# seagochen/unet-segment-pytorch

Hardware: AMD Instinct MI355X
Metric: 512x512 CT slices/sec fwd+bwd, AttentionUNet bs=4/GPU, 1/2/4/8 MI355X (higher is better)
Workload: dtype bf16; 1 GPU; attention_unet 1x512x512 train step (fwd+DiceBCE+bwd+clip+AdamW); model=attention_unet, global_batch=4, per_gpu_batch=4, grad_accum=1, parallelism=single

## Files before the change

### unet-segment-pytorch_amd/csrc/misc.hip

```cpp
#include "halo_items.h"

namespace unet {

__device__ __forceinline__ void up_range(float scale, int i, int in_size, int up, int& lo, int& hi) {
  if (scale > 0.f) {
    lo = (int)floorf((float)(i - 1) / scale) - 1;
    hi = (int)ceilf((float)(i + 1) / scale) + 1;
    lo = lo < 0 ? 0 : lo;
    hi = hi > up - 1 ? up - 1 : hi;
  } else {
    lo = 0;
    hi = up - 1;
  }
}
__device__ __forceinline__ float up_weight(float scale, int u, int in_size, int i) {
  int i0, i1;
  float l;
  lin_idx(scale, u, in_size, i0, i1, l);
  return (i0 == i ? 1.f - l : 0.f) + (i1 == i ? l : 0.f);
}

__global__ void upsample_bwd4_kernel(long long N, int C, int Hs, int Ws, int up_h, int up_w, int pt, int pl, int Hp,
                                     int Wp, float sh, float sw, const float* dup, float* dx, int accum) {
  const int C4 = C / 4;
// ... 93 lines not shown
                                                                int ntj, int ntc) {
  __shared__ float4 t[UPB_VMAX][UPB_CT];
  __shared__ int tab_i0[UPB_VMAX], tab_i1[UPB_VMAX];
  __shared__ float tab_l[UPB_VMAX];
  const int tid = threadIdx.x;
  const unsigned lb = xcd_block(blockIdx.x, gridDim.x);
  const int ct = (int)(lb % (unsigned)ntc);
  unsigned r = lb / (unsigned)ntc;
  const int jt = (int)(r % (unsigned)ntj);
  r /= (unsigned)ntj;
  const int i = (int)(r % (unsigned)Hs);
  const int n = (int)(r / (unsigned)Hs);
  const int C4 = C >> 2, c4 = ct * UPB_CT + (tid & (UPB_CT - 1));
  const int j0 = jt * UPB_J;
  const int ulo = max(0, (int)ceilf((float)(i - 1) / sh) - 1), uhi = min(up_h - 1, (int)floorf((float)(i + 1) / sh) + 1);
  float wy[8];
#pragma unroll
  for (int k = 0; k < 8; ++k) {
    const int u = ulo + k, yy = u + pt;
    wy[k] = (u <= uhi && yy >= 0 && yy < Hp) ? up_weight(sh, u, Hs, i) : 0.f;
  }
  const int jlast = min(Ws - 1, j0 + UPB_J - 1);
  const int vlo = max(0, (int)ceilf((float)(j0 - 1) / sw) - 1), vhi = min(up_w - 1, (int)floorf((float)(jlast + 1) / sw) + 1);
  const int nv = vhi - vlo + 1;
  if (tid < nv) {
    const int v = vlo + tid, xx = v + pl;
    int a0, a1;
    float l;
    lin_idx(sw, v, Ws, a0, a1, l);
    const bool ok = xx >= 0 && xx < Wp;
    tab_i0[tid] = ok ? a0 : -1;
    tab_i1[tid] = ok ? a1 : -1;
    tab_l[tid] = l;
  }
  const bool cok = c4 < C4;
  const size_t rowpix = (size_t)Wp * C4;
  const float4* base = reinterpret_cast<const float4*>(dup) + ((size_t)n * Hp + (ulo + pt)) * rowpix + c4;
  for (int it = tid >> 4; it < nv; it += 256 / UPB_CT) {
    const int xx = vlo + it + pl;
    float4 a = make_float4(0.f, 0.f, 0.f, 0.f);
    if (cok && xx >= 0 && xx < Wp) {
      const float4* p = base + (size_t)xx * C4;
      float4 g[8];
#pragma unroll
      for (int k = 0; k < 8; ++k) g[k] = wy[k] != 0.f ? p[(size_t)k * rowpix] : make_float4(0.f, 0.f, 0.f, 0.f);
#pragma unroll
      for (int k = 0; k < 8; ++k) {
        a.x = __builtin_fmaf(wy[k], g[k].x, a.x); a.y = __builtin_fmaf(wy[k], g[k].y, a.y);
        a.z = __builtin_fmaf(wy[k], g[k].z, a.z); a.w = __builtin_fmaf(wy[k], g[k].w, a.w);
      }
    }
    t[it][tid & (UPB_CT - 1)] = a;
  }
  __syncthreads();
  const int j = j0 + (tid >> 4);
  if (j > jlast || !cok) return;
  const int vjlo = max(vlo, (int)ceilf((float)(j - 1) / sw) - 1), vjhi = min(vhi, (int)floorf((float)(j + 1) / sw) + 1);
  float4 a = make_float4(0.f, 0.f, 0.f, 0.f);
  for (int v = vjlo; v <= vjhi; ++v) {
    const int q = v - vlo;
    const float l = tab_l[q];
    const float w = (tab_i0[q] == j ? 1.f - l : 0.f) + (tab_i1[q] == j ? l : 0.f);
    const float4 g = t[q][tid & (UPB_CT - 1)];
    a.x = __builtin_fmaf(w, g.x, a.x); a.y = __builtin_fmaf(w, g.y, a.y);
    a.z = __builtin_fmaf(w, g.z, a.z); a.w = __builtin_fmaf(w, g.w, a.w);
  }
  float4* o = reinterpret_cast<float4*>(dx) + (((size_t)n * Hs + i) * Ws + j) * C4 + c4;
  if (accum) {
    const float4 b = *o;
    a.x += b.x; a.y += b.y; a.z += b.z; a.w += b.w;
  }
  *o = a;
}

constexpr unsigned UPB_OOB = 0x40000000u;
typedef __amdgpu_buffer_rsrc_t upb_rsrc_t;
__device__ __forceinline__ upb_rsrc_t upb_rsrc(const void* p, unsigned bytes) {
  return __builtin_amdgcn_make_buffer_rsrc(const_cast<void*>(p), (short)0, (int)bytes, 0x00020000);
}
__device__ __forceinline__ uint4 upb_ld(upb_rsrc_t r, unsigned voff, unsigned soff) {
  return __builtin_bit_cast(uint4, __builtin_amdgcn_raw_buffer_load_b128(r, (int)voff, (int)soff, 0));
}

template <typename T, int NCH, int WA>
__global__ __launch_bounds__(256, 4) void upsample_bwd_pw_kernel(int N, int C, int Hs, int Ws, int up_h, int up_w, int pt,
                                                              int pl, int Hp, int Wp, float sh, float sw,
                                                              const float* __restrict__ dup,
                                                              const uint4* __restrict__ dgw,
                                                              const uint4* __restrict__ wt, float* dx, int accum,
                                                              int ntj, int ntc) {
  typedef typename Mma<T>::frag F;
  __shared__ float4 t[UPB_VMAX][UPB_CT + 1];
  __shared__ int tab_i0[UPB_VMAX], tab_i1[UPB_VMAX];
  __shared__ float tab_l[UPB_VMAX];
  const int tid = threadIdx.x, lane = tid & 63, wave = tid >> 6, i16 = lane & 15, g = lane >> 4;
  const unsigned lb = xcd_block(blockIdx.x, gridDim.x);
  const int ct = (int)(lb % (unsigned)ntc);
  unsigned r = lb / (unsigned)ntc;
  const int jt = (int)(r % (unsigned)ntj);
  r /= (unsigned)ntj;
  const int i = (int)(r % (unsigned)Hs);
  const int n = (int)(r / (unsigned)Hs);
  const int C4 = C >> 2;
  const int j0 = jt * UPB_J;
  const int ulo = max(0, (int)ceilf((float)(i - 1) / sh) - 1), uhi = min(up_h - 1, (int)floorf((float)(i + 1) / sh) + 1);
  float wy[8];
#pragma unroll
  for (int k = 0; k < 8; ++k) {
    const int u = ulo + k, yy = u + pt;
    wy[k] = (u <= uhi && yy >= 0 && yy < Hp) ? up_weight(sh, u, Hs, i) : 0.f;
  }
  const int jlast = min(Ws - 1, j0 + UPB_J - 1);
  const int vlo = max(0, (int)ceilf((float)(j0 - 1) / sw) - 1), vhi = min(up_w - 1, (int)floorf((float)(jlast + 1) / sw) + 1);
  const int nv = vhi - vlo + 1;
  if (tid < nv) {
    const int v = vlo + tid, xx = v + pl;
    int a0, a1;
    float l;
    lin_idx(sw, v, Ws, a0, a1, l);
    const bool ok = xx >= 0 && xx < Wp;
    tab_i0[tid] = ok ? a0 : -1;
    tab_i1[tid] = ok ? a1 : -1;
    tab_l[tid] = l;
  }
  const int wa = wave % (4 / WA), wg = wave / (4 / WA);
  F wq[WA][NCH];
#pragma unroll
  for (int aa = 0; aa < WA; ++aa)
#pragma unroll
    for (int c = 0; c < NCH; ++c)
      wq[aa][c] = __builtin_bit_cast(F, wt[((size_t)(ct * 4 + wa * WA + aa) * NCH + c) * 64 + lane]);
  const int cl = 4 * wa * WA + g;
  const size_t img = (size_t)Hp * Wp;
  const upb_rsrc_t dr = upb_rsrc(dup + (size_t)n * img * C, (unsigned)(img * C * 4));
  const upb_rsrc_t xr = upb_rsrc(dgw + (size_t)n * img * (4 * NCH), (unsigned)(img * (64 * NCH)));
  int nlive = 0, pos[8];
#pragma unroll
  for (int k = 0; k < 8; ++k) pos[k] = wy[k] != 0.f ? nlive++ : -1;
  float wl[8];
  unsigned rowd[8], rowx[8];
#pragma unroll
  for (int j = 0; j < 8; ++j) {
    wl[j] = 0.f;
    unsigned row = 0u;
#pragma unroll
    for (int k = 0; k < 8; ++k)
      if (pos[k] == j) { wl[j] = wy[k]; row = (unsigned)(ulo + k + pt) * (unsigned)Wp; }
    rowd[j] = row * (unsigned)C * 4u;
    rowx[j] = row * (unsigned)(64 * NCH);
  }
  const float4 z4 = make_float4(0.f, 0.f, 0.f, 0.f);
  for (int it = 16 * wg + i16; it - i16 < nv; it += 16 * WA) {
    const int xx = vlo + it + pl;
    const bool ok = it < nv && xx >= 0 && xx < Wp;
    const unsigned dvo = ok ? (unsigned)xx * (unsigned)C * 4u + (unsigned)(ct * UPB_CT + cl) * 16u : UPB_OOB;
    const unsigned xvo = ok ? (unsigned)xx * (unsigned)(64 * NCH) + (unsigned)g * 16u : UPB_OOB;
    float4 a[WA];
#pragma unroll
    for (int aa = 0; aa < WA; ++aa) a[aa] = z4;
#pragma unroll
    for (int k0 = 0; k0 < 8; k0 += 4) {
      if (k0 && nlive <= 4) break;
      float4 dv[WA][4];
      f32x4 acc[WA][4];
      unsigned dvk[4], xvk[4];
#pragma unroll
      for (int k = 0; k < 4; ++k) {
        const bool live = k0 + k < nlive;
        dvk[k] = live ? dvo : UPB_OOB;
        xvk[k] = live ? xvo : UPB_OOB;
#pragma unroll
        for (int aa = 0; aa < WA; ++aa) {
          dv[aa][k] = __builtin_bit_cast(float4, upb_ld(dr, dvk[k], rowd[k0 + k] + (unsigned)aa * 64u));
          acc[aa][k] = f32x4{0.f, 0.f, 0.f, 0.f};
        }
      }
#pragma unroll
      for (int c = 0; c < NCH; ++c) {
        uint4 q[4];
#pragma unroll
        for (int k = 0; k < 4; ++k) q[k] = upb_ld(xr, xvk[k], rowx[k0 + k] + (unsigned)c * 64u);
#pragma unroll
        for (int aa = 0; aa < WA; ++aa)
#pragma unroll
          for (int k = 0; k < 4; ++k)
            acc[aa][k] = Mma<T>::mma(wq[aa][c], __builtin_bit_cast(F, q[k]), acc[aa][k]);
      }
#pragma unroll
      for (int aa = 0; aa < WA; ++aa)
#pragma unroll
        for (int k = 0; k < 4; ++k) {
          float4 v = make_float4(acc[aa][k][0], acc[aa][k][1], acc[aa][k][2], acc[aa][k][3]);
          v.x += dv[aa][k].x; v.y += dv[aa][k].y; v.z += dv[aa][k].z; v.w += dv[aa][k].w;
          const float w = wl[k0 + k];
          a[aa].x = __builtin_fmaf(w, v.x, a[aa].x); a[aa].y = __builtin_fmaf(w, v.y, a[aa].y);
          a[aa].z = __builtin_fmaf(w, v.z, a[aa].z); a[aa].w = __builtin_fmaf(w, v.w, a[aa].w);
        }
    }
    if (it < nv) {
#pragma unroll
      for (int aa = 0; aa < WA; ++aa) t[it][cl + 4 * aa] = a[aa];
    }
  }
  __syncthreads();
  const int j = j0 + (tid >> 4);
  if (j > jlast) return;
  const int c4 = ct * UPB_CT + (tid & (UPB_CT - 1));
  const int vjlo = max(vlo, (int)ceilf((float)(j - 1) / sw) - 1), vjhi = min(vhi, (int)floorf((float)(j + 1) / sw) + 1);
  float4 a = z4;
  for (int v = vjlo; v <= vjhi; ++v) {
    const int q = v - vlo;
    const float l = tab_l[q];
    const float w = (tab_i0[q] == j ? 1.f - l : 0.f) + (tab_i1[q] == j ? l : 0.f);
    const float4 gq = t[q][tid & (UPB_CT - 1)];
    a.x = __builtin_fmaf(w, gq.x, a.x); a.y = __builtin_fmaf(w, gq.y, a.y);
    a.z = __builtin_fmaf(w, gq.z, a.z); a.w = __builtin_fmaf(w, gq.w, a.w);
  }
  float4* o = reinterpret_cast<float4*>(dx) + (((size_t)n * Hs + i) * Ws + j) * C4 + c4;
  if (accum) {
    const float4 b = *o;
    a.x += b.x; a.y += b.y; a.z += b.z; a.w += b.w;
  }
  *o = a;
}

template <typename T>
static void launch_upb_pw(int nch, unsigned nblk, hipStream_t st, int N, int C, int Hs, int Ws, int up_h, int up_w,
                          int pt, int pl, int Hp, int Wp, float sh, float sw, const float* d_up, const void* dgw,
                          const void* wt, float* dx, int accum, int ntj, int ntc) {
  const uint4* x = (const uint4*)dgw;
  const uint4* w = (const uint4*)wt;
  const char* e = getenv("UNET_GUP_WA");
  const int wa = e ? atoi(e) : 2;
#define UPB_PW_LAUNCH_WA(NCH, WA)                                                                                      \
  hipLaunchKernelGGL((upsample_bwd_pw_kernel<T, NCH, WA>), dim3(nblk), dim3(256), 0, st, N, C, Hs, Ws, up_h, up_w, pt, \
                     pl, Hp, Wp, sh, sw, d_up, x, w, dx, accum, ntj, ntc)
#define UPB_PW_LAUNCH(NCH)                   \
  do {                                       \
    if (wa == 2) UPB_PW_LAUNCH_WA(NCH, 2);   \
    else UPB_PW_LAUNCH_WA(NCH, 1);           \
  } while (0)
  if (nch == 1) UPB_PW_LAUNCH(1);
  else if (nch == 2) UPB_PW_LAUNCH(2);
  else if (nch == 4) UPB_PW_LAUNCH_WA(4, 1);
  else UPB_PW_LAUNCH_WA(8, 1);
#undef UPB_PW_LAUNCH
#undef UPB_PW_LAUNCH_WA
}

__global__ void upsample_bwd_kernel(long long N, int C, int Hs, int Ws, int up_h, int up_w, int pt, int pl, int Hp,
                                    int Wp, float sh, float sw, const float* dup, float* dx, int accum) {
  const long long total = N * Hs * (long long)Ws * C;
  for (long long e = blockIdx.x * (long long)blockDim.x + threadIdx.x; e < total; e += (long long)gridDim.x * blockDim.x) {
    const int c = e % C;
    long long t = e / C;
    const int j = t % Ws;
    t /= Ws;
    const int i = t % Hs;
    const long long n = t / Hs;
    int ulo, uhi, vlo, vhi;
    up_range(sh, i, Hs, up_h, ulo, uhi);
    up_range(sw, j, Ws, up_w, vlo, vhi);
    float acc = 0.f;
    for (int u = ulo; u <= uhi; ++u) {
      const float wy = up_weight(sh, u, Hs, i);
      if (wy == 0.f) continue;
      const int yy = u + pt;
      if (yy < 0 || yy >= Hp) continue;
      float racc = 0.f;
      for (int v = vlo; v <= vhi; ++v) {
        const float wx = up_weight(sw, v, Ws, j);
        if (wx == 0.f) continue;
        const int xx = v + pl;
        if (xx < 0 || xx >= Wp) continue;
        racc += wx * dup[((n * Hp + yy) * (long long)Wp + xx) * C + c];
      }
      acc += wy * racc;
    }
    dx[e] = accum ? dx[e] + acc : acc;
  }
}

__global__ void resize_nchw_kernel(long long NC, int Hi, int Wi, int Ho, int Wo, float sh, float sw, const float* x,
                                   float* y) {
  const long long total = NC * Ho * (long long)Wo;
  for (long long e = blockIdx.x * (long long)blockDim.x + threadIdx.x; e < total; e += (long long)gridDim.x * blockDim.x) {
    const int v = e % Wo;
    long long t = e / Wo;
    const int u = t % Ho;
    const long long nc = t / Ho;
    int y0, y1, x0, x1;
    float ly, lx;
    lin_idx(sh, u, Hi, y0, y1, ly);
    lin_idx(sw, v, Wi, x0, x1, lx);
    const float* p = x + nc * Hi * (long long)Wi;
    const float a = p[y0 * Wi + x0], b = p[y0 * Wi + x1], c = p[y1 * Wi + x0], d = p[y1 * Wi + x1];
    y[e] = (1.f - ly) * ((1.f - lx) * a + lx * b) + ly * ((1.f - lx) * c + lx * d);
  }
}

__global__ void resize_nchw_bwd_kernel(long long NC, int Hi, int Wi, int Ho, int Wo, float sh, float sw, const float* dy,
                                       float* dx, int accum) {
  const long long total = NC * Hi * (long long)Wi;
  for (long long e = blockIdx.x * (long long)blockDim.x + threadIdx.x; e < total; e += (long long)gridDim.x * blockDim.x) {
    const int j = e % Wi;
    long long t = e / Wi;
    const int i = t % Hi;
    const long long nc = t / Hi;
    int ulo, uhi, vlo, vhi;
    up_range(sh, i, Hi, Ho, ulo, uhi);
    up_range(sw, j, Wi, Wo, vlo, vhi);
    const float* p = dy + nc * Ho * (long long)Wo;
    float acc = 0.f;
    for (int u = ulo; u <= uhi; ++u) {
      const float wy = up_weight(sh, u, Hi, i);
      if (wy == 0.f) continue;
      float racc = 0.f;
      for (int v = vlo; v <= vhi; ++v) {
        const float wx = up_weight(sw, v, Wi, j);
        if (wx != 0.f) racc += wx * p[u * (long long)Wo + v];
      }
      acc += wy * racc;
    }
    dx[e] = accum ? dx[e] + acc : acc;
  }
}

constexpr int OC_MAXK = 8;

template <typename T>
// ... 649 lines not shown
  const I stride = (I)gridDim.x * blockDim.x;
  I e = (I)blockIdx.x * blockDim.x + threadIdx.x;
  const int cv = (int)(e & (CV - 1));
  float sc[VEC], sf[VEC];
#pragma unroll
  for (int j = 0; j < VEC; ++j) { sc[j] = s.scale[cv * VEC + j]; sf[j] = s.shift[cv * VEC + j]; }
  const float lo = s.relu ? 0.f : -INFINITY;
  for (; e < total; e += stride) {
    const I px = e >> cvs;
    const I t = px / (I)W;
    const int x = (int)(px - t * (I)W);
    const I t2 = t / (I)H;
    const int y = (int)(t - t2 * (I)H);
    const long long n = (long long)t2;
    float best[VEC];
    int arg[VEC];
#pragma unroll
    for (int q = 0; q < 4; ++q) {
      float v[VEC];
      load_vec<T>((const T*)s.data + (((n * s.H + 2 * y + (q >> 1)) * (long long)s.W + 2 * x + (q & 1)) * C + cv * VEC), v);
#pragma unroll
      for (int j = 0; j < VEC; ++j) {
        const float r = __builtin_fmaf(v[j], sc[j], sf[j]);
        const float a = r != r ? r : fmaxf(r, lo);
        if (q == 0 || a > best[j] || a != a) { best[j] = a; arg[j] = q; }
      }
    }
    store_vec<T>(out + (size_t)px * C + cv * VEC, best);
    unsigned lo4 = 0, hi4 = 0;
#pragma unroll
    for (int j = 0; j < 4; ++j) lo4 |= (unsigned)arg[j] << (8 * j);
    if constexpr (VEC == 8) {
#pragma unroll
      for (int j = 0; j < 4; ++j) hi4 |= (unsigned)arg[4 + j] << (8 * j);
      *reinterpret_cast<uint2*>(code + (size_t)px * C + cv * VEC) = make_uint2(lo4, hi4);
    } else {
      *reinterpret_cast<unsigned*>(code + (size_t)px * C + cv * VEC) = lo4;
    }
  }
}

}

using namespace unet;

extern "C" {

int unet_upsample_bwd(long long N, int C, int Hs, int Ws, int up_h, int up_w, int pad_t, int pad_l, int Hp, int Wp,
                      float sh, float sw, const float* d_up, float* dx, int accum, void* stream) {
  const long long total = N * Hs * (long long)Ws * C;
  auto span = [](float sc, int up) { return sc > 0.f ? (int)floorf(2.f / sc) + 3 : up + 8; };
  if (C % 4 == 0 && span(sh, up_h) <= 8 && span(sw, up_w) <= 8) {
    const int vspan = (int)floorf((float)(UPB_J + 1) / sw) + 4;
    const char* e = getenv("UNET_UPB_TILE");
    const long long ntj = cdiv(Ws, UPB_J), ntc = cdiv(C / 4, UPB_CT), nblk = N * Hs * ntj * ntc;
    if (!(e && atoi(e) == 0) && vspan <= UPB_VMAX && nblk < (1LL << 31)) {
      hipLaunchKernelGGL(upsample_bwd_tile_kernel, dim3((unsigned)nblk), dim3(256), 0, (hipStream_t)stream, (int)N, C, Hs,
                         Ws, up_h, up_w, pad_t, pad_l, Hp, Wp, sh, sw, d_up, dx, accum, (int)ntj, (int)ntc);
      return check_launch("upsample_bwd");
    }
    if (total / 4 < (1LL << 31))
      hipLaunchKernelGGL(upsample_bwd4w_kernel<unsigned>, dim3(grid_for(total / 4, block_cap("UNET_UPB_BLOCKS", 8192))), dim3(256), 0, (hipStream_t)stream,
                         N, C, Hs, Ws, up_h, up_w, pad_t, pad_l, Hp, Wp, sh, sw, d_up, dx, accum);
    else
      hipLaunchKernelGGL(upsample_bwd4w_kernel<unsigned long long>, dim3(grid_for(total / 4, block_cap("UNET_UPB_BLOCKS", 8192))), dim3(256), 0,
                         (hipStream_t)stream, N, C, Hs, Ws, up_h, up_w, pad_t, pad_l, Hp, Wp, sh, sw, d_up, dx, accum);
    return check_launch("upsample_bwd");
  }
  if (C % 4 == 0) {
    hipLaunchKernelGGL(upsample_bwd4_kernel, dim3(grid_for(total / 4, block_cap("UNET_UPB_BLOCKS", 8192))), dim3(256), 0, (hipStream_t)stream, N, C, Hs,
                       Ws, up_h, up_w, pad_t, pad_l, Hp, Wp, sh, sw, d_up, dx, accum);
    return check_launch("upsample_bwd");
  }
  hipLaunchKernelGGL(upsample_bwd_kernel, dim3(grid_for(total)), dim3(256), 0, (hipStream_t)stream, N, C, Hs, Ws,
                     up_h, up_w, pad_t, pad_l, Hp, Wp, sh, sw, d_up, dx, accum);
  return check_launch("upsample_bwd");
}

int unet_upsample_bwd_pw_ok(int dtype, long long N, int C, int Hs, int Ws, int up_h, int up_w, int pad_t, int pad_l,
                            int Hp, int Wp, float sh, float sw, int Ci) {
  if (dtype != UNET_BF16 && dtype != UNET_F16) return 0;
  if (N < 1 || C < 64 || C % 64 || (Ci != 32 && Ci != 64 && Ci != 128 && Ci != 256)) return 0;
  if (Hs < 1 || Ws < 1 || up_h < 1 || up_w < 1 || Hp < 1 || Wp < 1) return 0;
  auto span = [](float sc, int up) { return sc > 0.f ? (int)floorf(2.f / sc) + 3 : up + 8; };
  if (span(sh, up_h) > 8 || span(sw, up_w) > 8) return 0;
  const int vspan = (int)floorf((float)(UPB_J + 1) / sw) + 4;
  const char* e = getenv("UNET_UPB_TILE");
  const long long nblk = N * Hs * (long long)cdiv(Ws, UPB_J) * (C / 64);
  if ((e && atoi(e) == 0) || vspan > UPB_VMAX || nblk >= (1LL << 31) || N * Hs >= (1LL << 31)) return 0;
  const double img = (double)Hp * Wp;
  return img * C * 4 < (double)UPB_OOB && img * Ci * 2 < (double)UPB_OOB;
}

int unet_upsample_bwd_pw(int dtype, long long N, int C, int Hs, int Ws, int up_h, int up_w, int pad_t, int pad_l,
                         int Hp, int Wp, float sh, float sw, const float* d_up, const void* dgw, int Ci,
                         const void* wt_packed, float* dx, int accum, void* stream) {
  if (!unet_upsample_bwd_pw_ok(dtype, N, C, Hs, Ws, up_h, up_w, pad_t, pad_l, Hp, Wp, sh, sw, Ci)) {
    set_error("unet_upsample_bwd_pw: geometry not served (unet_upsample_bwd_pw_ok)");
    return -1;
  }
  const int ntj = cdiv(Ws, UPB_J), ntc = C / 64;
  const unsigned nblk = (unsigned)(N * Hs * ntj * ntc);
  if (dtype == UNET_F16)
    launch_upb_pw<f16>(Ci / 32, nblk, (hipStream_t)stream, (int)N, C, Hs, Ws, up_h, up_w, pad_t, pad_l, Hp, Wp, sh, sw,
                       d_up, dgw, wt_packed, dx, accum, ntj, ntc);
  else
    launch_upb_pw<bf16>(Ci / 32, nblk, (hipStream_t)stream, (int)N, C, Hs, Ws, up_h, up_w, pad_t, pad_l, Hp, Wp, sh, sw,
                        d_up, dgw, wt_packed, dx, accum, ntj, ntc);
  return check_launch("upsample_bwd_pw");
}

int unet_resize_nchw(long long NC, int Hi, int Wi, int Ho, int Wo, float sh, float sw, const float* x, float* y,
                     void* stream) {
  hipLaunchKernelGGL(resize_nchw_kernel, dim3(grid_for(NC * Ho * (long long)Wo)), dim3(256), 0, (hipStream_t)stream,
                     NC, Hi, Wi, Ho, Wo, sh, sw, x, y);
  return check_launch("resize_nchw");
}

int unet_resize_nchw_bwd(long long NC, int Hi, int Wi, int Ho, int Wo, float sh, float sw, const float* dy, float* dx,
                         int accum, void* stream) {
  hipLaunchKernelGGL(resize_nchw_bwd_kernel, dim3(grid_for(NC * Hi * (long long)Wi)), dim3(256), 0,
                     (hipStream_t)stream, NC, Hi, Wi, Ho, Wo, sh, sw, dy, dx, accum);
  return check_launch("resize_nchw_bwd");
}

int unet_outconv_rows(long long P) { return oc_rows(P); }

int unet_outconv_fwd(int dtype, long long N, int H, int W, int C, int K, const void* y, const float* scale,
                     const float* shift, int relu, const float* w, const float* b, float* logits, void* stream) {
  if (K > OC_MAXK || K < 1) { set_error("unet_outconv_fwd: n_classes > 8 unsupported"); return UNET_ERR_UNSUPPORTED; }
  const long long P = N * H * (long long)W;
  const int G = (C % 8 == 0 && C / 8 <= 64 && ((C / 8) & (C / 8 - 1)) == 0) ? C / 8 : 0;
  if (G && K == 2) {
    long long blocks = (P * G + 255) / 256;
    if (blocks > 4096) blocks = 4096;
    if (dtype == UNET_F16)
      hipLaunchKernelGGL((outconv_fwd_vec_kernel<f16, 2>), dim3((int)blocks), dim3(256), 0, (hipStream_t)stream, P,
                         H * W, C, G, (const f16*)y, scale, shift, relu, w, b, logits);
    else if (dtype == UNET_BF16)
      hipLaunchKernelGGL((outconv_fwd_vec_kernel<bf16, 2>), dim3((int)blocks), dim3(256), 0, (hipStream_t)stream, P,
                         H * W, C, G, (const bf16*)y, scale, shift, relu, w, b, logits);
    else
      hipLaunchKernelGGL((outconv_fwd_vec_kernel<float, 2>), dim3((int)blocks), dim3(256), 0, (hipStream_t)stream, P,
                         H * W, C, G, (const float*)y, scale, shift, relu, w, b, logits);
    return check_launch("outconv_fwd");
  }
  const size_t shm = (size_t)(K * C + 2 * C) * sizeof(float);
  if (dtype == UNET_F16)
    hipLaunchKernelGGL(outconv_fwd_kernel<f16>, dim3(grid_for(P)), dim3(256), shm, (hipStream_t)stream, P, H * W, C, K,
                       (const f16*)y, scale, shift, relu, w, b, logits);
  else if (dtype == UNET_BF16)
    hipLaunchKernelGGL(outconv_fwd_kernel<bf16>, dim3(grid_for(P)), dim3(256), shm, (hipStream_t)stream, P, H * W, C, K,
                       (const bf16*)y, scale, shift, relu, w, b, logits);
  else
    hipLaunchKernelGGL(outconv_fwd_kernel<float>, dim3(grid_for(P)), dim3(256), shm, (hipStream_t)stream, P, H * W, C,
                       K, (const float*)y, scale, shift, relu, w, b, logits);
  return check_launch("outconv_fwd");
}

int unet_outconv_bwd(int dtype, long long N, int H, int W, int C, int K, const void* y, const float* scale,
                     const float* shift, int relu, const float* w, const float* dl, float* da, int accum, float* partial,
                     void* stream) {
  if (K > OC_MAXK || K < 1 || C < K) { set_error("unet_outconv_bwd: need 1 <= n_classes <= min(8, C)"); return UNET_ERR_UNSUPPORTED; }
  const long long P = N * H * (long long)W;
  const int cl = chan_lanes_m(C), rows = oc_rows(P);
  const int G = (C % 8 == 0 && C / 8 <= 256 && ((C / 8) & (C / 8 - 1)) == 0) ? C / 8 : 0;
  if (dtype != UNET_F32 && G && K == 2) {
    if (dtype == UNET_F16)
      hipLaunchKernelGGL((outconv_bwd_vec_kernel<f16, 2>), dim3(rows), dim3(256), 0, (hipStream_t)stream, P, H * W, C, G,
                         (const f16*)y, scale, shift, relu, w, dl, da, accum, partial);
    else
      hipLaunchKernelGGL((outconv_bwd_vec_kernel<bf16, 2>), dim3(rows), dim3(256), 0, (hipStream_t)stream, P, H * W, C, G,
                         (const bf16*)y, scale, shift, relu, w, dl, da, accum, partial);
    return check_launch("outconv_bwd");
  }
  dim3 grid(cdiv(C, cl), rows);
  if (dtype == UNET_F16)
    hipLaunchKernelGGL(outconv_bwd_kernel<f16>, grid, dim3(256), 0, (hipStream_t)stream, P, H * W, C, cl, K,
                       (const f16*)y, scale, shift, relu, w, dl, da, accum, partial, rows);
  else if (dtype == UNET_BF16)
    hipLaunchKernelGGL(outconv_bwd_kernel<bf16>, grid, dim3(256), 0, (hipStream_t)stream, P, H * W, C, cl, K,
                       (const bf16*)y, scale, shift, relu, w, dl, da, accum, partial, rows);
  else
    hipLaunchKernelGGL(outconv_bwd_kernel<float>, grid, dim3(256), 0, (hipStream_t)stream, P, H * W, C, cl, K,
                       (const float*)y, scale, shift, relu, w, dl, da, accum, partial, rows);
  return check_launch("outconv_bwd");
}

int unet_outconv_bwd_bn(int dtype, long long N, int H, int W, int C, int K, const void* y, const float* scale,
                        const float* shift, int relu, const float* w, const float* dl, const float* mean,
                        const float* invstd, float* partial, float* bn_partial, void* stream) {
// ... 218 lines not shown
```

### unet-segment-pytorch_amd/unet/_hip/stages.py

```python

from __future__ import annotations

import os
from typing import Dict, List, Optional

import torch

from . import lib as L
from .runtime import (Act, Precision, conv_kernel_name, f32, pack_many, pack_weight, probe, stream, up_scale, vp,
                      wgrad_kernel_name)


def _conv_desc(prec: Precision, N: int, H: int, W: int, cin: int, cout: int, k: int, srcs: List[L.Src],
               weight: torch.Tensor) -> L.ConvDesc:
    d = L.ConvDesc()
    d.dtype = prec.code
    d.N, d.H, d.W, d.Cin, d.Cout, d.ksize = N, H, W, cin, cout, k
    d.nsrc = len(srcs)
    for i, s in enumerate(srcs):
        d.src[i] = s
    d.weight = weight.data_ptr()
    return d


# ... 311 lines not shown
        wg = self.cg.pre_wp if self.cg.pre_wp is not None else pack_weight(self.cg.conv.weight, prec, False)
        wx = self.cx.pre_wp if self.cx.pre_wp is not None else pack_weight(self.cx.conv.weight, prec, False)
        self.cg.pre_wp = self.cx.pre_wp = None
        gab, xab = f32(2, ci, device=dev), f32(2, ci, device=dev)
        for bn, ab in ((self.cg.bn, gab), (self.cx.bn, xab)):
            L.call("unet_bn_eval_affine", ci, vp(bn.weight), vp(bn.bias), vp(bn.running_mean), vp(bn.running_var),
                   float(bn.eps), vp(ab[0]), vp(ab[1]), None, None, stream())
        self.wpsi = self.psi_conv.weight.detach().reshape(-1).float().contiguous()
        self.p = f32(x.N, x.H, x.W, device=dev)
        L.call("unet_gate_psi_eval", prec.code, x.pixels, g_up_t.shape[-1], x.C, ci, vp(g_up_t), vp(x.data),
               vp(x.ab[0]), vp(x.ab[1]), int(x.relu), vp(wg), vp(wx), vp(gab), vp(xab), vp(self.wpsi),
               vp(self.p), stream())
        bn = self.psi_bn
        self.psi_ab = f32(2, 1, device=dev)
        L.call("unet_bn_eval_affine", 1, vp(bn.weight), vp(bn.bias), vp(bn.running_mean), vp(bn.running_var),
               float(bn.eps), vp(self.psi_ab[0]), vp(self.psi_ab[1]), None, None, stream())

    def gated_src(self) -> L.Src:
        return self.x.src_gated(self.p, self.psi_ab)

    def backward(self, prec, d_xs: torch.Tensor, grads: Grads, d_gup: Optional[torch.Tensor], d_gup_accum: int,
                 defer_g: bool = False):
        x = self.x
        dev = x.data.device
        P, Cx, Ci = x.pixels, x.C, self.ci
        fuse = self._wx_gated_ok(prec, x)
        dx, dx_acc = (None, 0) if fuse else x.grad_target()
        dq = f32(P, device=dev)
        rows1 = L.load().unet_gate_psi_rows(P)
        part1 = f32(2, rows1, device=dev)
        L.call("unet_gate_bwd1", prec.code, P, Cx, vp(d_xs), vp(x.data), vp(x.ab[0]), vp(x.ab[1]), int(x.relu), vp(self.p),
               vp(self.psi_ab), vp(self.psi_mean), vp(self.psi_invstd), vp(dx), dx_acc, vp(dq), vp(part1), stream())
        dgp, dbp, pcoef = f32(1, device=dev), f32(1, device=dev), f32(3, device=dev)
        L.call("unet_bn_bwd_finalize", vp(part1[0]), vp(part1[1]), rows1, 1, P if self.psi_batch else 0,
               vp(self.psi_bn.weight),
               vp(self.psi_mean), vp(self.psi_invstd), vp(dgp), vp(dbp), 0, vp(pcoef), stream())
        grads.put(self.psi_bn.weight, dgp)
        grads.put(self.psi_bn.bias, dbp)
        rows2 = L.load().unet_gate_bwd2_rows(P, Ci)
        part2 = f32(4, rows2, Ci, device=dev)
        L.call("unet_gate_bwd2", prec.code, P, Ci, vp(self.gw.data), vp(self.xw.data), vp(self.gw.ab),
               vp(self.xw.ab), vp(self.gw.mean), vp(self.gw.invstd), vp(self.xw.mean), vp(self.xw.invstd),
               vp(self.wpsi), vp(dq), vp(self.p), vp(pcoef), vp(part2), stream())
        dgg, dbg, gcoef = f32(Ci, device=dev), f32(Ci, device=dev), f32(3, Ci, device=dev)
        dgx, dbx, xcoef = f32(Ci, device=dev), f32(Ci, device=dev), f32(3, Ci, device=dev)
        dwpsi = f32(Ci, device=dev)
        jobs = [_bwd_fin_job(part2[0], part2[1], rows2, Ci, P if self.gw.batch_stats else 0, self.cg.bn.weight,
                             self.gw.mean, self.gw.invstd, dgg, dbg, gcoef),
                _bwd_fin_job(part2[0], part2[2], rows2, Ci, P if self.xw.batch_stats else 0, self.cx.bn.weight,
                             self.xw.mean, self.xw.invstd, dgx, dbx, xcoef),
                _bwd_fin_job(part2[3], None, rows2, Ci, 0, None, None, None, None, dwpsi, None)]
        L.call("unet_bn_bwd_finalize_multi", len(jobs), (L.BnBwdFinJob * len(jobs))(*jobs), stream())
        grads.put(self.cg.bn.weight, dgg)
        grads.put(self.cg.bn.bias, dbg)
        grads.put(self.cx.bn.weight, dgx)
        grads.put(self.cx.bn.bias, dbx)
        grads.put(self.psi_conv.weight, dwpsi.view(1, Ci, 1, 1))
        dgw = torch.empty(x.N, x.H, x.W, Ci, dtype=prec.torch_dtype, device=dev)
        dxw = torch.empty_like(dgw)
        L.call("unet_gate_bwd3", prec.code, P, Ci, vp(self.gw.data), vp(self.xw.data), vp(self.gw.ab),
               vp(self.xw.ab), vp(self.wpsi), vp(dq), vp(self.p), vp(pcoef), vp(gcoef), vp(xcoef), vp(dgw), vp(dxw),
               stream())
        wt_g = None
        if defer_g:
            wt_g = self.cg.pre_wt if self.cg.pre_wt is not None else pack_weight(self.cg.conv.weight, prec,
                                                                                 transpose=True)
            self.cg.pre_wt = None
            self.cg.conv_backward(prec, dgw, self.gw_src, grads, None)
        else:
            self.cg.conv_backward(prec, dgw, self.gw_src, grads,
                                  {"mode": "f32", "out": d_gup, "accum": d_gup_accum})
        dx2, acc2 = x.grad_target()
        if fuse:
            self.cx.conv_backward(prec, dxw, [x.src()], grads, {"mode": "f32_gated", "out": dx2, "accum": acc2,
                                                                "dxs": d_xs, "gate_p": self.p,
                                                                "gate_ab": self.psi_ab})
        else:
            self.cx.conv_backward(prec, dxw, [x.src()], grads, {"mode": "f32", "out": dx2, "accum": acc2})
        return (dgw, wt_g) if defer_g else None

    def up_fused_ok(self, prec, g: Act, x: Act) -> bool:
        if prec.code not in (L.BF16, L.F16) or os.environ.get("UNET_NO_GUP_FUSE"):
            return False
        if self.ci > 64 and not os.environ.get("UNET_GUP_DEEP"):
            return False
        d = L.ConvDesc()
        d.dtype, d.N, d.H, d.W, d.Cin, d.Cout, d.ksize, d.nsrc = prec.code, x.N, x.H, x.W, self.ci, g.C, 1, 1
        s = L.Src()
        s.kind, s.C, s.H, s.W = L.SRC_PLAIN, self.ci, x.H, x.W
        d.src[0] = s
        d.out_mode, d.split, d.accum = L.OUT_F32, g.C, 1
        if not conv_kernel_name(d).startswith("pw_conv_kernel"):
            return False
        return bool(L.load().unet_upsample_bwd_pw_ok(prec.code, g.N, g.C, g.H, g.W, x.H, x.W, 0, 0, x.H, x.W,
                                                     up_scale(g.H, x.H), up_scale(g.W, x.W), self.ci))

    def _wx_gated_ok(self, prec, x: Act) -> bool:
        if prec.code not in (L.BF16, L.F16) or os.environ.get("UNET_NO_GATE_FUSE"):
            return False
        d = L.ConvDesc()
        d.dtype, d.N, d.H, d.W, d.Cin, d.Cout, d.ksize, d.nsrc = prec.code, x.N, x.H, x.W, self.ci, x.C, 1, 1
        s = L.Src()
        s.kind, s.C, s.H, s.W = L.SRC_PLAIN, self.ci, x.H, x.W
        d.src[0] = s
        d.out_mode, d.split = L.OUT_F32_GATED, x.C
        return conv_kernel_name(d).startswith("pw_conv_kernel")


def mark_tracked(stage, tracked: bool):
    for attr in ("c1", "c2", "cg", "cx"):
        cb = getattr(stage, attr, None)
        if cb is not None:
            cb.tracked = tracked
    for attr in ("dc", "gate"):
        sub = getattr(stage, attr, None)
        if sub is not None:
            mark_tracked(sub, tracked)


def _pad_geometry(x1: Act, x2: Act):
    up_h, up_w = 2 * x1.H, 2 * x1.W
    dy, dx = x2.H - up_h, x2.W - up_w
    return up_h, up_w, dy // 2, dx // 2


class ConvTStage:

    def __init__(self, m: torch.nn.ConvTranspose2d):
        if m.kernel_size != (2, 2) or m.stride != (2, 2) or m.padding != (0, 0) or m.groups != 1 or \
                m.dilation != (1, 1) or m.output_padding != (0, 0):
            raise NotImplementedError("unet HIP path: only ConvTranspose2d(k=2, s=2) is supported")
        self.m = m
        self.cin, self.ct = m.in_channels, m.out_channels

    def _w4(self) -> torch.Tensor:
        return self.m.weight.detach().float().permute(2, 3, 1, 0).reshape(4 * self.ct, self.cin, 1, 1).contiguous()

    def forward(self, prec, x1: Act) -> Act:
        dev = x1.data.device
        N, h, w = x1.N, x1.H, x1.W
        self.x1 = x1
        self.w4 = self._w4()
        wp = pack_weight(self.w4, prec, transpose=False)
        y = torch.empty(N, 2 * h, 2 * w, self.ct, dtype=prec.torch_dtype, device=dev)
        d = _conv_desc(prec, N, h, w, self.cin, 4 * self.ct, 1, [x1.src()], wp)
        d.out_mode = L.OUT_SHUFFLE2
        d.out = y.data_ptr()
        b = self.m.bias
        self.bias = b.detach().float().contiguous() if b is not None else None
        d.bias = vp(self.bias)
        probe.launch(lambda: conv_kernel_name(d), 2.0 * N * h * w * self.cin * 4 * self.ct,
                     lambda: L.call("unet_conv", d, stream()), d.out_mode)
        return Act(y, None, False)

    def backward(self, prec, d_up: torch.Tensor, pad_t: int, pad_l: int, grads: Grads, need_dx: bool = True):
        x1 = self.x1
        dev = x1.data.device
        N, h, w, ct = x1.N, x1.H, x1.W, self.ct
        P = N * h * w
        dys = torch.empty(N, h, w, 4 * ct, dtype=prec.torch_dtype, device=dev)
        rows = L.load().unet_convt_bwd_rows(P)
        part = f32(rows, ct, device=dev)
        L.call("unet_convt_bwd_prep", prec.code, N, h, w, ct, d_up.shape[1], d_up.shape[2], pad_t, pad_l, vp(d_up),
               vp(dys), vp(part), stream())
        if self.m.bias is not None:
            db = f32(ct, device=dev)
            L.call("unet_colsum", vp(part), rows, ct, vp(db), 0, stream())
# ... 317 lines not shown
```

Baseline: 513.5 img/s.

## Tile upsample-backward pointwise kernel over multiple output rows with prefetched stages

The fused upsample-backward pointwise kernel now processes R output rows per block and shares each loaded source row's MMA result across all rows it feeds, using a ballot mask of live rows. Loads for the next stage are double-buffered, and the column tile width becomes a template parameter (24 or 16). The Python gate now enables the fused path for deeper channel counts and skips only very small spatial sizes. This cuts redundant loads and MMAs for overlapping rows, at the cost of more registers, lower occupancy bounds and more template instantiations.

```diff
diff --git a/unet-segment-pytorch_amd/csrc/misc.hip b/unet-segment-pytorch_amd/csrc/misc.hip
--- a/unet-segment-pytorch_amd/csrc/misc.hip
+++ b/unet-segment-pytorch_amd/csrc/misc.hip
@@ -199,35 +199,27 @@
   return __builtin_bit_cast(uint4, __builtin_amdgcn_raw_buffer_load_b128(r, (int)voff, (int)soff, 0));
 }
 
-template <typename T, int NCH, int WA>
-__global__ __launch_bounds__(256, 4) void upsample_bwd_pw_kernel(int N, int C, int Hs, int Ws, int up_h, int up_w, int pt,
-                                                              int pl, int Hp, int Wp, float sh, float sw,
-                                                              const float* __restrict__ dup,
-                                                              const uint4* __restrict__ dgw,
-                                                              const uint4* __restrict__ wt, float* dx, int accum,
-                                                              int ntj, int ntc) {
+template <typename T, int NCH, int WA, int R, int J, int RB, int OCC>
+__global__ __launch_bounds__(256, OCC) void upsample_bwd_pw_kernel(
+    int N, int C, int Hs, int Ws, int up_h, int up_w, int pt, int pl, int Hp, int Wp, float sh, float sw,
+    const float* __restrict__ dup, const uint4* __restrict__ dgw, const uint4* __restrict__ wt, float* dx, int accum,
+    int ntj, int ntc) {
   typedef typename Mma<T>::frag F;
-  __shared__ float4 t[UPB_VMAX][UPB_CT + 1];
+  __shared__ float4 t[R][UPB_VMAX][UPB_CT + 1];
   __shared__ int tab_i0[UPB_VMAX], tab_i1[UPB_VMAX];
   __shared__ float tab_l[UPB_VMAX];
   const int tid = threadIdx.x, lane = tid & 63, wave = tid >> 6, i16 = lane & 15, g = lane >> 4;
   const unsigned lb = xcd_block(blockIdx.x, gridDim.x);
   const int ct = (int)(lb % (unsigned)ntc);
-  unsigned r = lb / (unsigned)ntc;
-  const int jt = (int)(r % (unsigned)ntj);
-  r /= (unsigned)ntj;
-  const int i = (int)(r % (unsigned)Hs);
-  const int n = (int)(r / (unsigned)Hs);
+  unsigned rr = lb / (unsigned)ntc;
+  const int jt = (int)(rr % (unsigned)ntj);
+  rr /= (unsigned)ntj;
+  const unsigned ngr = ((unsigned)Hs + R - 1) / R;
+  const int ibase = (int)(rr % ngr) * R;
+  const int n = (int)(rr / ngr);
   const int C4 = C >> 2;
-  const int j0 = jt * UPB_J;
-  const int ulo = max(0, (int)ceilf((float)(i - 1) / sh) - 1), uhi = min(up_h - 1, (int)floorf((float)(i + 1) / sh) + 1);
-  float wy[8];
-#pragma unroll
-  for (int k = 0; k < 8; ++k) {
-    const int u = ulo + k, yy = u + pt;
-    wy[k] = (u <= uhi && yy >= 0 && yy < Hp) ? up_weight(sh, u, Hs, i) : 0.f;
-  }
-  const int jlast = min(Ws - 1, j0 + UPB_J - 1);
+  const int j0 = jt * J;
+  const int jlast = min(Ws - 1, j0 + J - 1);
   const int vlo = max(0, (int)ceilf((float)(j0 - 1) / sw) - 1), vhi = min(up_w - 1, (int)floorf((float)(jlast + 1) / sw) + 1);
   const int nv = vhi - vlo + 1;
   if (tid < nv) {
@@ -240,6 +232,20 @@
     tab_i1[tid] = ok ? a1 : -1;
     tab_l[tid] = l;
   }
+  const int U0 = max(0, (int)ceilf((float)(ibase - 1) / sh) - 1);
+  float wr[R];
+  bool feeds = false;
+  {
+    const int u = U0 + lane, yy = u + pt;
+#pragma unroll
+    for (int r = 0; r < R; ++r) {
+      const int i = ibase + r;
+      const int ulo = max(0, (int)ceilf((float)(i - 1) / sh) - 1), uhi = min(up_h - 1, (int)floorf((float)(i + 1) / sh) + 1);
+      wr[r] = (i < Hs && u >= ulo && u <= uhi && yy >= 0 && yy < Hp) ? up_weight(sh, u, Hs, i) : 0.f;
+      feeds = feeds || wr[r] != 0.f;
+    }
+  }
+  const unsigned long long live = __ballot(feeds);
   const int wa = wave % (4 / WA), wg = wave / (4 / WA);
   F wq[WA][NCH];
 #pragma unroll
@@ -251,118 +257,142 @@
   const size_t img = (size_t)Hp * Wp;
   const upb_rsrc_t dr = upb_rsrc(dup + (size_t)n * img * C, (unsigned)(img * C * 4));
   const upb_rsrc_t xr = upb_rsrc(dgw + (size_t)n * img * (4 * NCH), (unsigned)(img * (64 * NCH)));
-  int nlive = 0, pos[8];
-#pragma unroll
-  for (int k = 0; k < 8; ++k) pos[k] = wy[k] != 0.f ? nlive++ : -1;
-  float wl[8];
-  unsigned rowd[8], rowx[8];
-#pragma unroll
-  for (int j = 0; j < 8; ++j) {
-    wl[j] = 0.f;
-    unsigned row = 0u;
-#pragma unroll
-    for (int k = 0; k < 8; ++k)
-      if (pos[k] == j) { wl[j] = wy[k]; row = (unsigned)(ulo + k + pt) * (unsigned)Wp; }
-    rowd[j] = row * (unsigned)C * 4u;
-    rowx[j] = row * (unsigned)(64 * NCH);
-  }
   const float4 z4 = make_float4(0.f, 0.f, 0.f, 0.f);
   for (int it = 16 * wg + i16; it - i16 < nv; it += 16 * WA) {
     const int xx = vlo + it + pl;
     const bool ok = it < nv && xx >= 0 && xx < Wp;
     const unsigned dvo = ok ? (unsigned)xx * (unsigned)C * 4u + (unsigned)(ct * UPB_CT + cl) * 16u : UPB_OOB;
     const unsigned xvo = ok ? (unsigned)xx * (unsigned)(64 * NCH) + (unsigned)g * 16u : UPB_OOB;
-    float4 a[WA];
-#pragma unroll
-    for (int aa = 0; aa < WA; ++aa) a[aa] = z4;
-#pragma unroll
-    for (int k0 = 0; k0 < 8; k0 += 4) {
-      if (k0 && nlive <= 4) break;
-      float4 dv[WA][4];
-      f32x4 acc[WA][4];
-      unsigned dvk[4], xvk[4];
-#pragma unroll
-      for (int k = 0; k < 4; ++k) {
-        const bool live = k0 + k < nlive;
-        dvk[k] = live ? dvo : UPB_OOB;
-        xvk[k] = live ? xvo : UPB_OOB;
+    float4 a[R][WA];
+#pragma unroll
+    for (int r = 0; r < R; ++r)
+#pragma unroll
+      for (int aa = 0; aa < WA; ++aa) a[r][aa] = z4;
+    float4 dv[RB][WA], dvn[RB][WA];
+    uint4 q[RB][NCH], qn[RB][NCH];
+    int sl[RB], sln[RB];
+    unsigned long long m = live;
+#define UPB_STAGE_LOAD(DV, Q, SL)                                                                                   \
+  _Pragma("unroll") for (int k = 0; k < RB; ++k) {                                                              \
+    SL[k] = m ? (int)__builtin_ctzll(m) : -1;                                                                       \
+    m &= m - 1ull;                                                                                                  \
+    const unsigned row = SL[k] < 0 ? 0u : (unsigned)(U0 + SL[k] + pt) * (unsigned)Wp;                               \
+    const unsigned dk = SL[k] < 0 ? UPB_OOB : dvo, xk = SL[k] < 0 ? UPB_OOB : xvo;                                  \
+    _Pragma("unroll") for (int aa = 0; aa < WA; ++aa)                                                               \
+        DV[k][aa] = __builtin_bit_cast(float4, upb_ld(dr, dk, row * (unsigned)C * 4u + (unsigned)aa * 64u));        \
+    _Pragma("unroll") for (int c = 0; c < NCH; ++c)                                                                 \
+        Q[k][c] = upb_ld(xr, xk, row * (unsigned)(64 * NCH) + (unsigned)c * 64u);                                   \
+  }
+    UPB_STAGE_LOAD(dv, q, sl)
+    while (sl[0] >= 0) {
+      UPB_STAGE_LOAD(dvn, qn, sln)
+#pragma unroll
+      for (int k = 0; k < RB; ++k) {
+        if (sl[k] < 0) continue;
+        f32x4 acc[WA];
+#pragma unroll
+        for (int aa = 0; aa < WA; ++aa) acc[aa] = f32x4{0.f, 0.f, 0.f, 0.f};
+#pragma unroll
+        for (int c = 0; c < NCH; ++c)
+#pragma unroll
+          for (int aa = 0; aa < WA; ++aa) acc[aa] = Mma<T>::mma(wq[aa][c], __builtin_bit_cast(F, q[k][c]), acc[aa]);
+        float4 v[WA];
 #pragma unroll
         for (int aa = 0; aa < WA; ++aa) {
-          dv[aa][k] = __builtin_bit_cast(float4, upb_ld(dr, dvk[k], rowd[k0 + k] + (unsigned)aa * 64u));
-          acc[aa][k] = f32x4{0.f, 0.f, 0.f, 0.f};
+          v[aa] = make_float4(acc[aa][0], acc[aa][1], acc[aa][2], acc[aa][3]);
+          v[aa].x += dv[k][aa].x; v[aa].y += dv[k][aa].y; v[aa].z += dv[k][aa].z; v[aa].w += dv[k][aa].w;
         }
-      }
-#pragma unroll
-      for (int c = 0; c < NCH; ++c) {
-        uint4 q[4];
-#pragma unroll
-        for (int k = 0; k < 4; ++k) q[k] = upb_ld(xr, xvk[k], rowx[k0 + k] + (unsigned)c * 64u);
-#pragma unroll
-        for (int aa = 0; aa < WA; ++aa)
-#pragma unroll
-          for (int k = 0; k < 4; ++k)
-            acc[aa][k] = Mma<T>::mma(wq[aa][c], __builtin_bit_cast(F, q[k]), acc[aa][k]);
-      }
-#pragma unroll
-      for (int aa = 0; aa < WA; ++aa)
-#pragma unroll
-        for (int k = 0; k < 4; ++k) {
-          float4 v = make_float4(acc[aa][k][0], acc[aa][k][1], acc[aa][k][2], acc[aa][k][3]);
-          v.x += dv[aa][k].x; v.y += dv[aa][k].y; v.z += dv[aa][k].z; v.w += dv[aa][k].w;
-          const float w = wl[k0 + k];
-          a[aa].x = __builtin_fmaf(w, v.x, a[aa].x); a[aa].y = __builtin_fmaf(w, v.y, a[aa].y);
-          a[aa].z = __builtin_fmaf(w, v.z, a[aa].z); a[aa].w = __builtin_fmaf(w, v.w, a[aa].w);
+#pragma unroll
+        for (int r = 0; r < R; ++r) {
+          const float w = __builtin_bit_cast(float, __builtin_amdgcn_readlane(__builtin_bit_cast(int, wr[r]), sl[k]));
+          if (w == 0.f) continue;
+#pragma unroll
+          for (int aa = 0; aa < WA; ++aa) {
+            a[r][aa].x = __builtin_fmaf(w, v[aa].x, a[r][aa].x); a[r][aa].y = __builtin_fmaf(w, v[aa].y, a[r][aa].y);
+            a[r][aa].z = __builtin_fmaf(w, v[aa].z, a[r][aa].z); a[r][aa].w = __builtin_fmaf(w, v[aa].w, a[r][aa].w);
+          }
         }
-    }
+      }
+#pragma unroll
+      for (int k = 0; k < RB; ++k) {
+        sl[k] = sln[k];
+#pragma unroll
+        for (int aa = 0; aa < WA; ++aa) dv[k][aa] = dvn[k][aa];
+#pragma unroll
+        for (int c = 0; c < NCH; ++c) q[k][c] = qn[k][c];
+      }
+    }
+#undef UPB_STAGE_LOAD
     if (it < nv) {
 #pragma unroll
-      for (int aa = 0; aa < WA; ++aa) t[it][cl + 4 * aa] = a[aa];
+      for (int r = 0; r < R; ++r)
+#pragma unroll
+        for (int aa = 0; aa < WA; ++aa) t[r][it][cl + 4 * aa] = a[r][aa];
     }
   }
   __syncthreads();
-  const int j = j0 + (tid >> 4);
-  if (j > jlast) return;
-  const int c4 = ct * UPB_CT + (tid & (UPB_CT - 1));
-  const int vjlo = max(vlo, (int)ceilf((float)(j - 1) / sw) - 1), vjhi = min(vhi, (int)floorf((float)(j + 1) / sw) + 1);
-  float4 a = z4;
-  for (int v = vjlo; v <= vjhi; ++v) {
-    const int q = v - vlo;
-    const float l = tab_l[q];
-    const float w = (tab_i0[q] == j ? 1.f - l : 0.f) + (tab_i1[q] == j ? l : 0.f);
-    const float4 gq = t[q][tid & (UPB_CT - 1)];
-    a.x = __builtin_fmaf(w, gq.x, a.x); a.y = __builtin_fmaf(w, gq.y, a.y);
-    a.z = __builtin_fmaf(w, gq.z, a.z); a.w = __builtin_fmaf(w, gq.w, a.w);
-  }
-  float4* o = reinterpret_cast<float4*>(dx) + (((size_t)n * Hs + i) * Ws + j) * C4 + c4;
-  if (accum) {
-    const float4 b = *o;
-    a.x += b.x; a.y += b.y; a.z += b.z; a.w += b.w;
-  }
-  *o = a;
+  const int cv = tid & (UPB_CT - 1), c4 = ct * UPB_CT + cv;
+  for (int j = j0 + (tid >> 4); j <= jlast; j += 256 / UPB_CT) {
+    const int vjlo = max(vlo, (int)ceilf((float)(j - 1) / sw) - 1), vjhi = min(vhi, (int)floorf((float)(j + 1) / sw) + 1);
+    float4 a[R];
+#pragma unroll
+    for (int r = 0; r < R; ++r) a[r] = z4;
+    for (int v = vjlo; v <= vjhi; ++v) {
+      const int qi = v - vlo;
+      const float l = tab_l[qi];
+      const float w = (tab_i0[qi] == j ? 1.f - l : 0.f) + (tab_i1[qi] == j ? l : 0.f);
+#pragma unroll
+      for (int r = 0; r < R; ++r) {
+        const float4 gq = t[r][qi][cv];
+        a[r].x = __builtin_fmaf(w, gq.x, a[r].x); a[r].y = __builtin_fmaf(w, gq.y, a[r].y);
+        a[r].z = __builtin_fmaf(w, gq.z, a[r].z); a[r].w = __builtin_fmaf(w, gq.w, a[r].w);
+      }
+    }
+#pragma unroll
+    for (int r = 0; r < R; ++r) {
+      if (ibase + r >= Hs) break;
+      float4* o = reinterpret_cast<float4*>(dx) + (((size_t)n * Hs + ibase + r) * Ws + j) * C4 + c4;
+      float4 s = a[r];
+      if (accum) {
+        const float4 b = *o;
+        s.x += b.x; s.y += b.y; s.z += b.z; s.w += b.w;
+      }
+      *o = s;
+    }
+  }
+}
+
+static int upb_vspan(int J, float sw) { return (int)floorf((float)(J + 1) / sw) + 4; }
+
+template <typename T, int NCH, int WA, int R, int J, int RB, int OCC>
+static void launch_upb_pw_tile(hipStream_t st, int N, int C, int Hs, int Ws, int up_h, int up_w, int pt, int pl, int Hp,
+                               int Wp, float sh, float sw, const float* d_up, const void* dgw, const void* wt, float* dx,
+                               int accum) {
+  const int ntj = cdiv(Ws, J), ntc = C / 64;
+  const unsigned nblk = (unsigned)((long long)N * cdiv(Hs, R) * ntj * ntc);
+  hipLaunchKernelGGL((upsample_bwd_pw_kernel<T, NCH, WA, R, J, RB, OCC>), dim3(nblk), dim3(256), 0, st, N, C, Hs, Ws,
+                     up_h, up_w, pt, pl, Hp, Wp, sh, sw, d_up, (const uint4*)dgw, (const uint4*)wt, dx, accum, ntj, ntc);
 }
 
 template <typename T>
-static void launch_upb_pw(int nch, unsigned nblk, hipStream_t st, int N, int C, int Hs, int Ws, int up_h, int up_w,
-                          int pt, int pl, int Hp, int Wp, float sh, float sw, const float* d_up, const void* dgw,
-                          const void* wt, float* dx, int accum, int ntj, int ntc) {
-  const uint4* x = (const uint4*)dgw;
-  const uint4* w = (const uint4*)wt;
-  const char* e = getenv("UNET_GUP_WA");
-  const int wa = e ? atoi(e) : 2;
-#define UPB_PW_LAUNCH_WA(NCH, WA)                                                                                      \
-  hipLaunchKernelGGL((upsample_bwd_pw_kernel<T, NCH, WA>), dim3(nblk), dim3(256), 0, st, N, C, Hs, Ws, up_h, up_w, pt, \
-                     pl, Hp, Wp, sh, sw, d_up, x, w, dx, accum, ntj, ntc)
-#define UPB_PW_LAUNCH(NCH)                   \
-  do {                                       \
-    if (wa == 2) UPB_PW_LAUNCH_WA(NCH, 2);   \
-    else UPB_PW_LAUNCH_WA(NCH, 1);           \
-  } while (0)
-  if (nch == 1) UPB_PW_LAUNCH(1);
-  else if (nch == 2) UPB_PW_LAUNCH(2);
-  else if (nch == 4) UPB_PW_LAUNCH_WA(4, 1);
-  else UPB_PW_LAUNCH_WA(8, 1);
-#undef UPB_PW_LAUNCH
-#undef UPB_PW_LAUNCH_WA
+static void launch_upb_pw(int nch, hipStream_t st, int N, int C, int Hs, int Ws, int up_h, int up_w, int pt, int pl,
+                          int Hp, int Wp, float sh, float sw, const float* d_up, const void* dgw, const void* wt,
+                          float* dx, int accum) {
+#define UPB_ARGS st, N, C, Hs, Ws, up_h, up_w, pt, pl, Hp, Wp, sh, sw, d_up, dgw, wt, dx, accum
+  const bool j24 = upb_vspan(24, sw) <= UPB_VMAX;
+  if (nch == 1) {
+    if (j24) launch_upb_pw_tile<T, 1, 2, 2, 24, 2, 4>(UPB_ARGS);
+    else launch_upb_pw_tile<T, 1, 2, 2, 16, 2, 4>(UPB_ARGS);
+  } else if (nch == 2) {
+    if (j24) launch_upb_pw_tile<T, 2, 4, 4, 24, 1, 2>(UPB_ARGS);
+    else launch_upb_pw_tile<T, 2, 4, 4, 16, 1, 2>(UPB_ARGS);
+  } else if (nch == 4) {
+    if (j24) launch_upb_pw_tile<T, 4, 4, 4, 24, 1, 2>(UPB_ARGS);
+    else launch_upb_pw_tile<T, 4, 4, 4, 16, 1, 2>(UPB_ARGS);
+  } else {
+    launch_upb_pw_tile<T, 8, 2, 4, 16, 1, 2>(UPB_ARGS);
+  }
+#undef UPB_ARGS
 }
 
 __global__ void upsample_bwd_kernel(long long N, int C, int Hs, int Ws, int up_h, int up_w, int pt, int pl, int Hp,
@@ -1178,7 +1208,7 @@
   if (dtype != UNET_BF16 && dtype != UNET_F16) return 0;
   if (N < 1 || C < 64 || C % 64 || (Ci != 32 && Ci != 64 && Ci != 128 && Ci != 256)) return 0;
   if (Hs < 1 || Ws < 1 || up_h < 1 || up_w < 1 || Hp < 1 || Wp < 1) return 0;
-  auto span = [](float sc, int up) { return sc > 0.f ? (int)floorf(2.f / sc) + 3 : up + 8; };
+  auto span = [](float sc, int up) { return sc > 0.f ? min(up, (int)floorf(2.f / sc) + 3) : up + 8; };
   if (span(sh, up_h) > 8 || span(sw, up_w) > 8) return 0;
   const int vspan = (int)floorf((float)(UPB_J + 1) / sw) + 4;
   const char* e = getenv("UNET_UPB_TILE");
@@ -1195,14 +1225,12 @@
     set_error("unet_upsample_bwd_pw: geometry not served (unet_upsample_bwd_pw_ok)");
     return -1;
   }
-  const int ntj = cdiv(Ws, UPB_J), ntc = C / 64;
-  const unsigned nblk = (unsigned)(N * Hs * ntj * ntc);
   if (dtype == UNET_F16)
-    launch_upb_pw<f16>(Ci / 32, nblk, (hipStream_t)stream, (int)N, C, Hs, Ws, up_h, up_w, pad_t, pad_l, Hp, Wp, sh, sw,
-                       d_up, dgw, wt_packed, dx, accum, ntj, ntc);
+    launch_upb_pw<f16>(Ci / 32, (hipStream_t)stream, (int)N, C, Hs, Ws, up_h, up_w, pad_t, pad_l, Hp, Wp, sh, sw, d_up, dgw,
+                       wt_packed, dx, accum);
   else
-    launch_upb_pw<bf16>(Ci / 32, nblk, (hipStream_t)stream, (int)N, C, Hs, Ws, up_h, up_w, pad_t, pad_l, Hp, Wp, sh, sw,
-                        d_up, dgw, wt_packed, dx, accum, ntj, ntc);
+    launch_upb_pw<bf16>(Ci / 32, (hipStream_t)stream, (int)N, C, Hs, Ws, up_h, up_w, pad_t, pad_l, Hp, Wp, sh, sw, d_up, dgw,
+                        wt_packed, dx, accum);
   return check_launch("upsample_bwd_pw");
 }
 
diff --git a/unet-segment-pytorch_amd/unet/_hip/stages.py b/unet-segment-pytorch_amd/unet/_hip/stages.py
--- a/unet-segment-pytorch_amd/unet/_hip/stages.py
+++ b/unet-segment-pytorch_amd/unet/_hip/stages.py
@@ -417,7 +417,7 @@
     def up_fused_ok(self, prec, g: Act, x: Act) -> bool:
         if prec.code not in (L.BF16, L.F16) or os.environ.get("UNET_NO_GUP_FUSE"):
             return False
-        if self.ci > 64 and not os.environ.get("UNET_GUP_DEEP"):
+        if min(x.H, x.W) <= 8:
             return False
         d = L.ConvDesc()
         d.dtype, d.N, d.H, d.W, d.Cin, d.Cout, d.ksize, d.nsrc = prec.code, x.N, x.H, x.W, self.ci, g.C, 1, 1
```

Measured after the change: 519.3 img/s (median of 6 runs). 1.1% higher.
